# AI4Science-WestlakeU/safediffcon

Measured on AMD Instinct MI355X. Metric: sampled control trajectories/sec (1000-step DDPM), higher is better.
Workload: dtype f32; 1 GPU; C4: 2D smoke Unet3D_with_Conv3D dim=64 (1,2,4) state (B,32,7,64,64), B=64 per GPU, guided 1000-step DDPM, conformal quantile on; batch_per_gpu=64, global_batch=64, step=U-Net + guidance + posterior update of the whole batch, one hipGraph replay, parallelism=batch-sharded x1, no data-path collective, conv_precision=fp32

## Files before the change

include/sdc.h:

```cpp
#ifndef SDC_H
#define SDC_H

#include <stddef.h>
#include <stdint.h>

#ifdef __cplusplus
extern "C" {
#endif

#define SDC_OK 0
#define SDC_EINVAL (-1)
#define SDC_EALIGN (-2)
#define SDC_EHIP (-3)
#define SDC_ENULL (-4)

int sdc_version(void);
int sdc_last_error(char* buf, size_t cap);

typedef struct SdcConvDesc {
    int32_t B, Cin0, Cin1, Cout;
    int32_t iD, iH, iW;
    int32_t oD, oH, oW;
    int32_t kD, kH, kW;
    int32_t sD, sH, sW;
// ... 138 lines not shown
    int32_t pD, pH, pW;
    int32_t uD, uH, uW;
    int32_t precision;
    int64_t gs[5], xs[5];
} SdcWgradDesc;
size_t sdc_conv_wgrad_bytes(const SdcWgradDesc* d);
int sdc_conv_wgrad(const SdcWgradDesc* d, const float* g, const float* x, float* dw, float* dbias, void* work,
                   size_t work_bytes, void* stream);

#define SDC_F16_EXP_INTS 1025
int sdc_f16_grad_exponent(const float* g, int B, int C, int D, int H, int W, const int64_t* strides, int32_t* e, void* stream);

int sdc_conv_dgrad_f16(const SdcConvDesc* d, const float* g, const float* wp, const int32_t* e, float* dx, void* stream);

size_t sdc_conv_wgrad_f16_bytes(const SdcWgradDesc* d);
int sdc_conv_wgrad_f16(const SdcWgradDesc* d, const float* g, const float* x, const int32_t* e, float* dw, float* dbias, void* work,
                       size_t work_bytes, void* stream);
int sdc_conv_wgrad_describe(const SdcWgradDesc* d, char* name, size_t cap);

int sdc_conv_stem_f16_ok(const SdcConvDesc* d);
size_t sdc_pack_stem_f16_bytes(int Cout, int Cin, int kD, int kH, int kW);
int sdc_pack_stem_f16(const float* w, void* out, int Cout, int Cin, int kD, int kH, int kW, void* stream);
int sdc_conv_stem_f16(const SdcConvDesc* d, const float* x, const void* wh, const float* bias, float* y, void* stream);

int sdc_conv_stem_x3_ok(const SdcConvDesc* d);
size_t sdc_pack_stem_x3_bytes(int Cout, int Cin, int kD, int kH, int kW);
int sdc_pack_stem_x3(const float* w, void* out, int Cout, int Cin, int kD, int kH, int kW, void* stream);
int sdc_conv_stem_x3(const SdcConvDesc* d, const float* x, const void* wb, const float* bias, float* y, void* stream);

int sdc_conv_gemm_x3_ok(const SdcConvDesc* d);
size_t sdc_pack_gemm_x3_bytes(int Cout, int Cin, int kH, int kW);
int sdc_pack_gemm_x3(const float* wp, void* out, int Cout, int Cin, int kH, int kW, void* stream);
int sdc_conv_gemm_x3(const SdcConvDesc* d, const float* x, const void* wb, const float* bias, float* y, void* stream);

int sdc_conv_wino3_x3_ok(const SdcConvDesc* d);
size_t sdc_pack_wino3_x3_bytes(int Cout, int Cin);
int sdc_pack_wino3_x3(const float* wp, void* out, int Cout, int Cin, void* stream);
int sdc_conv_wino3_x3(const SdcConvDesc* d, const float* x, const float* x1, const void* wb, const float* bias, float* y,
                      double* gn_parts, int gn_groups, void* stream);

size_t sdc_gn_silu_bwd_floats(int B, int C, int G, int64_t S);
int sdc_gn_silu_bwd(const float* h, const float* gy, const float* stats, const float* gamma, const float* beta,
                    const float* ss, int64_t ss_b_stride, float* rows, float* gh, float* dgamma, float* dbeta, float* dss,
                    int B, int C, int G, int64_t S, void* stream);

size_t sdc_chan_norm_bwd_parts(int B, int64_t S);
size_t sdc_chan_norm_bwd_bytes(int B, int C, int64_t S);
int sdc_chan_norm_bwd(const float* x, const float* gy, const float* g, float* gx, float* gpart, int B, int C, int64_t S,
                      int mode, float eps, void* stream);

size_t sdc_pack_conv_weight_floats(int Cout, int Cin, int kD, int kH, int kW, int precision);
int sdc_pack_conv_weight(const float* w, float* out, int Cout, int Cin, int kD, int kH, int kW, int precision, int flip, void* stream);

typedef struct SdcPackItem {
    const float* w;
    float* out;
    int Cout, Cin, kD, kH, kW, precision, flip;
    int co_sh, ci_sh, grid_x, grid_y, block0;
    unsigned tap_magic;
    int64_t n[5];
} SdcPackItem;
int sdc_pack_batch_plan(SdcPackItem* items, int n, int* total_blocks, int* lds_bytes);
int sdc_pack_batch_run(const SdcPackItem* items_dev, int n, int total_blocks, int lds_bytes, void* stream);

size_t sdc_attn_bwd_bytes(int outer, int inner, int heads, int ntok);
int sdc_attn_bwd(const float* qkv, const float* dout, const float* rot, const float* bias, float* dqkv, float* dbias, void* work,
// ... 108 lines not shown
```

safediffcon_amd/_lib.py:

```python
import ctypes as C
import os

_HERE = os.path.dirname(os.path.abspath(__file__))
LIB_PATH = os.path.join(_HERE, "libsdc_hip.so")

SDC_MODEL_BURGERS, SDC_MODEL_TOKAMAK, SDC_MODEL_SMOKE = 0, 1, 2

_f32p = C.c_void_p
_i32p = C.c_void_p
_stream = C.c_void_p
_i64 = C.c_int64


class SdcConvDesc(C.Structure):
    _fields_ = [(n, C.c_int32) for n in (
        "B", "Cin0", "Cin1", "Cout", "iD", "iH", "iW", "oD", "oH", "oW", "kD", "kH", "kW", "sD", "sH", "sW",
        "pD", "pH", "pW", "uD", "uH", "uW", "up_mode", "precision")] + [
        ("x0s", C.c_int64 * 5), ("x1s", C.c_int64 * 5), ("ys", C.c_int64 * 5), ("rs", C.c_int64 * 5)]


class SdcStepDesc(C.Structure):
    _fields_ = [(n, C.c_int32) for n in (
        "model", "B", "d0", "d1", "d2", "d3", "guide", "clip", "impose", "cond_idx", "pad_zero", "use_max",
        "has_wgt", "skip_draws", "ddim")] + [("_pad", C.c_int32), ("seed", C.c_uint64)]
# ... 85 lines not shown
    "sdc_pack_tattn_x3": (C.c_int, [_f32p, _f32p, C.c_void_p, _stream]),
    "sdc_tattn_block_x3": (C.c_int, [_f32p, _f32p, C.c_void_p, _f32p, _f32p, _f32p, C.c_int, C.c_int, C.c_int, C.c_int,
                                     _i64, _i64, _i64, C.c_float, _stream]),
    "sdc_tattn_block_x3_ok": (C.c_int, [C.c_int, C.c_int, C.c_int]),
    "sdc_attn": (C.c_int, [_f32p, _f32p, _f32p, _f32p, C.c_int, C.c_int, C.c_int, C.c_int, _i64, _i64, _i64, _i64,
                           _i64, _i64, _i64, _i64, _stream]),
    "sdc_act": (C.c_int, [_f32p, _f32p, _i64, C.c_int, _stream]),
    "sdc_guide_reduce": (C.c_int, [C.POINTER(SdcStepDesc), _f32p, _f32p, _f32p, _i32p, _f32p, _f32p, _stream]),
    "sdc_step_update": (C.c_int, [C.POINTER(SdcStepDesc), _f32p, _f32p, _f32p, _f32p, _i32p, _i32p, _f32p, _i64,
                                  _f32p, _f32p, _f32p, _f32p, _f32p, _f32p, _f32p, _f32p, _stream]),
    "sdc_impose": (C.c_int, [C.POINTER(SdcStepDesc), _f32p, _f32p, _f32p, _f32p, _stream]),
    "sdc_randn": (C.c_int, [_f32p, _i64, C.c_uint64, _i32p, _stream]),
    "sdc_advance": (C.c_int, [_i32p, C.c_int, _i32p, C.c_int, _stream]),
    "sdc_advance_table": (C.c_int, [_i32p, _i32p, _i32p, _i32p, C.c_int, _stream]),
    "sdc_conformal_score": (C.c_int, [C.POINTER(SdcStepDesc), _f32p, _f32p, _f32p, _f32p, _f32p, _f32p, _stream]),
    "sdc_burgers_rollout": (C.c_int, [_f32p, _f32p, _f32p, C.c_int, C.c_int, C.c_int, C.c_int, C.c_int, C.c_float, C.c_float,
                                      C.c_float, C.c_float, C.c_float, _stream]),
    "sdc_conv_wgrad_bytes": (C.c_size_t, [C.POINTER(SdcWgradDesc)]),
    "sdc_conv_wgrad": (C.c_int, [C.POINTER(SdcWgradDesc), _f32p, _f32p, _f32p, _f32p, C.c_void_p, C.c_size_t, _stream]),
    "sdc_f16_grad_exponent": (C.c_int, [_f32p, C.c_int, C.c_int, C.c_int, C.c_int, C.c_int, C.c_void_p, C.c_void_p, _stream]),
    "sdc_conv_dgrad_f16": (C.c_int, [C.POINTER(SdcConvDesc), _f32p, _f32p, C.c_void_p, _f32p, _stream]),
    "sdc_conv_stem_f16_ok": (C.c_int, [C.POINTER(SdcConvDesc)]),
    "sdc_pack_stem_f16_bytes": (C.c_size_t, [C.c_int, C.c_int, C.c_int, C.c_int, C.c_int]),
    "sdc_pack_stem_f16": (C.c_int, [_f32p, C.c_void_p, C.c_int, C.c_int, C.c_int, C.c_int, C.c_int, _stream]),
    "sdc_conv_stem_f16": (C.c_int, [C.POINTER(SdcConvDesc), _f32p, C.c_void_p, _f32p, _f32p, _stream]),
    "sdc_conv_stem_x3_ok": (C.c_int, [C.POINTER(SdcConvDesc)]),
    "sdc_pack_stem_x3_bytes": (C.c_size_t, [C.c_int, C.c_int, C.c_int, C.c_int, C.c_int]),
    "sdc_pack_stem_x3": (C.c_int, [_f32p, C.c_void_p, C.c_int, C.c_int, C.c_int, C.c_int, C.c_int, _stream]),
    "sdc_conv_stem_x3": (C.c_int, [C.POINTER(SdcConvDesc), _f32p, C.c_void_p, _f32p, _f32p, _stream]),
    "sdc_conv_gemm_x3_ok": (C.c_int, [C.POINTER(SdcConvDesc)]),
    "sdc_pack_gemm_x3_bytes": (C.c_size_t, [C.c_int, C.c_int, C.c_int, C.c_int]),
    "sdc_pack_gemm_x3": (C.c_int, [_f32p, C.c_void_p, C.c_int, C.c_int, C.c_int, C.c_int, _stream]),
    "sdc_conv_gemm_x3": (C.c_int, [C.POINTER(SdcConvDesc), _f32p, C.c_void_p, _f32p, _f32p, _stream]),
    "sdc_conv_wino3_x3_ok": (C.c_int, [C.POINTER(SdcConvDesc)]),
    "sdc_pack_wino3_x3_bytes": (C.c_size_t, [C.c_int, C.c_int]),
    "sdc_pack_wino3_x3": (C.c_int, [_f32p, C.c_void_p, C.c_int, C.c_int, _stream]),
    "sdc_conv_wino3_x3": (C.c_int, [C.POINTER(SdcConvDesc), _f32p, _f32p, C.c_void_p, _f32p, _f32p, C.c_void_p, C.c_int, _stream]),
    "sdc_conv_wgrad_f16_bytes": (C.c_size_t, [C.POINTER(SdcWgradDesc)]),
    "sdc_conv_wgrad_f16": (C.c_int, [C.POINTER(SdcWgradDesc), _f32p, _f32p, C.c_void_p, _f32p, _f32p, C.c_void_p, C.c_size_t, _stream]),
    "sdc_conv_wgrad_describe": (C.c_int, [C.POINTER(SdcWgradDesc), C.c_char_p, C.c_size_t]),
    "sdc_gn_silu_bwd_floats": (C.c_size_t, [C.c_int, C.c_int, C.c_int, _i64]),
    "sdc_gn_silu_bwd": (C.c_int, [_f32p, _f32p, _f32p, _f32p, _f32p, _f32p, _i64, _f32p, _f32p, _f32p, _f32p, _f32p,
                                  C.c_int, C.c_int, C.c_int, _i64, _stream]),
    "sdc_chan_norm_bwd_parts": (C.c_size_t, [C.c_int, _i64]),
    "sdc_chan_norm_bwd_bytes": (C.c_size_t, [C.c_int, C.c_int, _i64]),
    "sdc_chan_norm_bwd": (C.c_int, [_f32p, _f32p, _f32p, _f32p, _f32p, C.c_int, C.c_int, _i64, C.c_int, C.c_float, _stream]),
    "sdc_pack_conv_weight_floats": (C.c_size_t, [C.c_int, C.c_int, C.c_int, C.c_int, C.c_int, C.c_int]),
    "sdc_pack_conv_weight": (C.c_int, [_f32p, _f32p, C.c_int, C.c_int, C.c_int, C.c_int, C.c_int, C.c_int, C.c_int, _stream]),
    "sdc_pack_batch_plan": (C.c_int, [C.POINTER(SdcPackItem), C.c_int, C.POINTER(C.c_int), C.POINTER(C.c_int)]),
    "sdc_pack_batch_run": (C.c_int, [C.c_void_p, C.c_int, C.c_int, C.c_int, _stream]),
    "sdc_attn_bwd_bytes": (C.c_size_t, [C.c_int, C.c_int, C.c_int, C.c_int]),
    "sdc_attn_bwd": (C.c_int, [_f32p, _f32p, _f32p, _f32p, _f32p, _f32p, C.c_void_p, C.c_int, C.c_int, C.c_int, C.c_int,
                               _i64, _i64, _i64, _i64, _i64, _i64, _i64, _i64, _stream]),
    "sdc_linattn_bwd_bytes": (C.c_size_t, [C.c_int, C.c_int, C.c_int, _i64]),
    "sdc_linattn_bwd": (C.c_int, [_f32p, _f32p, _f32p, C.c_void_p, C.c_int, C.c_int, C.c_int, _i64, _i64, _i64, _i64, _i64, _i64, _i64,
                                  _stream]),
    "sdc_act_bwd": (C.c_int, [_f32p, _f32p, _f32p, _i64, C.c_int, _stream]),
    "sdc_sumpool2": (C.c_int, [_f32p, _f32p, _i64, C.c_int, C.c_int, C.c_int, C.c_int, _stream]),
    "sdc_kstar_lstm_floats": (C.c_size_t, []),
    "sdc_kstar_rollout": (C.c_int, [C.POINTER(SdcKstarModel), _f32p, _i64, _i64, _i64, C.c_void_p, C.c_void_p, C.c_int, C.c_int, _stream]),
    "sdc_smoke_rollout_workspace_bytes": (C.c_size_t, [C.c_int]),
    "sdc_smoke_rollout": (C.c_int, [_f32p, _f32p, _i64, _i64, _f32p, _i64, _f32p, _i64, C.c_void_p, C.c_void_p, C.c_void_p,
                                    C.c_int, C.c_int, C.c_void_p, C.c_void_p, C.c_void_p, C.c_size_t, C.c_int, C.c_int, C.c_int,
                                    C.c_int, C.c_int, C.c_int, C.c_double, C.c_int, _stream]),
    "sdc_conv_splitk_bytes": (C.c_size_t, [C.POINTER(SdcConvDesc)]),
    "sdc_conv_splitk": (C.c_int, [C.POINTER(SdcConvDesc), _f32p, _f32p, _f32p, _f32p, _f32p, _f32p, C.c_size_t, _stream]),
# ... 57 lines not shown
```

safediffcon_amd/build.py:

```python
import os
import subprocess
import sys

HERE = os.path.dirname(os.path.abspath(__file__))
CSRC = os.path.join(HERE, "csrc")
LIB = os.path.join(HERE, "libsdc_hip.so")
SOURCES = ["sdc_api.hip", "sdc_conv.hip", "sdc_conv_wino.hip", "sdc_conv_f16.hip", "sdc_conv_stem_f16.hip", "sdc_conv_stem_x3.hip", "sdc_conv_gemm_x3.hip", "sdc_conv_wino_x3.hip", "sdc_norm.hip", "sdc_attn.hip", "sdc_lablock.hip", "sdc_lablock_f16.hip", "sdc_lablock_x3.hip", "sdc_tablock.hip", "sdc_tablock_f16.hip", "sdc_tablock_x3.hip", "sdc_step.hip", "sdc_solver.hip", "sdc_grad.hip", "sdc_wgrad_f16.hip", "sdc_attn_bwd.hip", "sdc_kstar.hip", "sdc_smoke.hip", "sdc_linear.hip", "sdc_optim.hip"]
HEADERS = ["sdc_common.h", "sdc_lablock_tile.h", "sdc_tablock_tile.h", "sdc_conv_stem_tile.h", "sdc_split3.h", "sdc_f16frag.h", "sdc_conv.h", "sdc_conv_wino3s.inc", "sdc_conv_wino2s.inc", "sdc_conv_pw2.inc"]
HIPCC = os.environ.get("HIPCC", "/opt/rocm/bin/hipcc")
FLAGS = ["--offload-arch=gfx950", "-O3", "-fPIC", "-std=c++17", "-Wall", "-Wno-unused-function"]


def source_hash():
    import hashlib
    h = hashlib.sha256()
    for f in SOURCES + HEADERS:
        with open(os.path.join(CSRC, f), "rb") as fh:
            h.update(fh.read())
    with open(os.path.join(HERE, "..", "include", "sdc.h"), "rb") as fh:
        h.update(fh.read())
    return h.hexdigest()[:16]


def _stale(out, deps):
    if not os.path.exists(out):
        return True
    t = os.path.getmtime(out)
    return any(os.path.getmtime(d) > t for d in deps)


def build_experiments(verbose=True):
    out = os.path.join(HERE, "libsdc_hip_exp.so")
    cmd = [HIPCC, *FLAGS, "-DSDC_KERNEL_EXPERIMENTS", "-shared", *[os.path.join(CSRC, s) for s in SOURCES], "-o", out]
    if verbose:
        print(" ".join(cmd), flush=True)
    subprocess.check_call(cmd)
    return out


def build(force=False, verbose=True, jobs=4):
# ... 28 lines not shown
```

safediffcon_amd/csrc/sdc_conv.h:

```cpp
#pragma once
#include "sdc_common.h"
#include <cstdlib>
#include <type_traits>

namespace sdcconv {


#ifdef SDC_KERNEL_EXPERIMENTS
inline int exp_env(const char* name) { const char* v = getenv(name); return v ? atoi(v) : 0; }
#else
constexpr int exp_env(const char*) { return 0; }
#endif


constexpr int BK = 16;
constexpr int NT = 256;

typedef float f32x16 __attribute__((ext_vector_type(16)));

typedef const __attribute__((address_space(1))) float* gfloat_p;
__device__ __forceinline__ gfloat_p uniform_ptr(const float* p) {
    const uint64_t u = reinterpret_cast<uint64_t>(p);
    const uint32_t lo = __builtin_amdgcn_readfirstlane((uint32_t)u);
    const uint32_t hi = __builtin_amdgcn_readfirstlane((uint32_t)(u >> 32));
// ... 38 lines not shown
constexpr int W3S_TILES = 32;

inline int64_t span5(const int64_t* st, int b, int c, int dd, int h, int w) {
    return (int64_t)(b - 1) * st[0] + (int64_t)(c - 1) * st[1] + (int64_t)(dd - 1) * st[2] + (int64_t)(h - 1) * st[3] + (int64_t)(w - 1) * st[4];
}

bool wg2_ok(const SdcConvDesc& d, bool small);
bool wg3_ok(const SdcConvDesc& d, bool small);
int launch_wg2(const ConvArgs& a, hipStream_t s);
int wg2_ksplit(const SdcConvDesc& d);
int launch_wg3(const ConvArgs& a, hipStream_t s);
bool wg3s_ok(const SdcConvDesc& d, bool small);
bool wg2s_ok(const SdcConvDesc& d, bool small);
int launch_wg2s(const ConvArgs& a, hipStream_t s);
int launch_wg3s(const ConvArgs& a, hipStream_t s);

int f16_kc(int kD, int kH, int kW);
bool f16_faster(const SdcConvDesc& d);
bool f16_ok(const SdcConvDesc& d);
int f16_gnparts(const SdcConvDesc& d, int G);
const char* f16_name(const SdcConvDesc& d);
int launch_f16(const ConvArgs& a, const _Float16* wh, hipStream_t s, const int32_t* gexp = nullptr);
int pack_f16_tail(const float* w, float* tail, int64_t gap, int Cout, int Cin, int kD, int kH, int kW, hipStream_t s);

struct StemShape { int Hs, NG, NR, itemsB; size_t lds; };
StemShape stem_shape(const SdcConvDesc& d);
int launch_stem_f16(const SdcConvDesc& d, const float* x, const _Float16* wh, const float* bias, float* y, hipStream_t s);

int launch_stem_x3(const SdcConvDesc& d, const float* x, const __bf16* wb, const float* bias, float* y, hipStream_t s);

bool gemm_x3_covers(const SdcConvDesc& d);
int launch_gemm_x3(const SdcConvDesc& d, const float* x, const __bf16* wb, const float* bias, float* y, hipStream_t s);

}
```

safediffcon_amd/csrc/sdc_conv.hip:

```cpp
#include "sdc_conv.h"
#include <string>

using namespace sdcconv;

namespace {

template <int TM, int TN>
__device__ __forceinline__ void conv_epilogue(const ConvArgs& a, f32x16 (&acc)[TM][TN], int mw, int nw, int lane, float* ybase = nullptr) {
    const SdcConvDesc& d = a.d;
    float* const ay = ybase ? ybase : a.y;
    const int l31 = lane & 31, lh = lane >> 5;
    if (a.ydense && mw + TM * 32 <= d.Cout) {
        typedef __attribute__((address_space(1))) char* gwchar_p;
        typedef __attribute__((address_space(1))) float* gwfloat_p;
        typedef const __attribute__((address_space(1))) char* gchar_p;
        const int S = d.oD * d.oH * d.oW;
        const float r_S = 1.0f / (float)S;
        const int64_t ycs4 = d.ys[1] * 4, rcs4 = d.rs[1] * 4;
        uint32_t yoff[TN], roff[TN];
        bool pok[TN];
#pragma unroll
        for (int j = 0; j < TN; ++j) {
            const int pp = nw + j * 32 + l31;
            pok[j] = pp < a.Ntot;
// ... 1474 lines not shown
        return (int64_t)(b - 1) * st[0] + (int64_t)(dd - 1) * st[2] + (int64_t)(h - 1) * st[3] + (int64_t)(w - 1) * st[4];
    };
    return span(d.x0s, d.B, d.iD, d.iH, d.iW) < (1ll << 30) && (d.Cin1 == 0 || span(d.x1s, d.B, d.iD, d.iH, d.iW) < (1ll << 30));
}

bool y_dense(const SdcConvDesc& d, bool residual) {
    auto dense = [&](const int64_t* st) { return st[4] == 1 && st[3] == d.oW && st[2] == (int64_t)d.oH * d.oW; };
    const int64_t S = (int64_t)d.oD * d.oH * d.oW;
    return dense(d.ys) && S >= 128 && S < (1 << 24) && span5(d.ys, d.B, d.Cout, d.oD, d.oH, d.oW) < (1ll << 30) &&
           (!residual || (dense(d.rs) && span5(d.rs, d.B, d.Cout, d.oD, d.oH, d.oW) < (1ll << 30)));
}

struct Operands { const void *x0, *x1, *wp, *y, *res; };
const void* const ALIGNED = reinterpret_cast<const void*>(uintptr_t(256));
const Operands CANONICAL{ALIGNED, ALIGNED, ALIGNED, ALIGNED, nullptr};

bool aligned(const void* p, int bytes) { return reinterpret_cast<uintptr_t>(p) % bytes == 0; }

bool wino_aligned(const SdcConvDesc& d, const Operands& op, bool stores) {
    return aligned(op.wp, 16) && aligned(op.x0, 16) && (d.Cin1 == 0 || aligned(op.x1, 16)) && (!stores || (aligned(op.y, 8) && !op.res));
}

std::string wino_misfit(const SdcConvDesc& d, const Operands& op) {
    std::string s;
    auto add = [&](bool miss, const char* what) { if (miss) s += (s.empty() ? "" : ", ") + std::string(what); };
    add(!aligned(op.wp, 16), "wp is not 16-byte aligned");
    add(!aligned(op.x0, 16), "x0 is not 16-byte aligned");
    add(d.Cin1 > 0 && !aligned(op.x1, 16), "x1 is not 16-byte aligned");
    add(!aligned(op.y, 8), "y is not 8-byte aligned");
    add(op.res != nullptr, "a residual is fused");
    return s.empty() ? "the operands differ from the descriptor-only assumption" : s;
}

enum class Kern { F16, WG3S, WG3, WG2S, WG2, WG1, PW2, PW, STEM, DIRECT };
struct Route {
    Kern kern;
    const char* name;
    double share;
    int gn_parts;
    int ksplit;
    bool sum_bias;
    int tile;
    bool ups;
    Direct form;
};

Route make_route(Kern k, const char* name, double share, int gn_parts = 0, int tile = 0) {
    return Route{k, name, share, gn_parts, 1, false, tile, false, Direct::GEN};
}

Route route(const SdcConvDesc& d, const Operands& op, int G, bool split) {
    if (d.precision == 6 || d.precision == 7) {
        if (!split && f16_ok(d)) return make_route(Kern::F16, f16_name(d), 1.0, f16_gnparts(d, G));
        SdcConvDesc d4 = d;
        d4.precision = 4;
        return route(d4, op, G, split);
    }
    const bool small = conv_small(d);
    const int64_t ntot = (int64_t)d.B * d.oD * d.oH * d.oW;
    const bool splits = split && !op.res;
    if (wg3s_ok(d, small) && wino_aligned(d, op, true))
        return make_route(Kern::WG3S, d.oW == 16 ? "conv_wg3s_kernel<16>" : (d.oW == 32 ? "conv_wg3s_kernel<32>" : "conv_wg3s_kernel<64>"),
                          8.0 / 27.0, gn_parts_for(d, W2_BM, W3S_TILES * 8, G));
    if (wg3_ok(d, small) && wino_aligned(d, op, true))
        return make_route(Kern::WG3, d.oW == 16 ? "conv_wg3_kernel<16>" : (d.oW == 32 ? "conv_wg3_kernel<32>" : "conv_wg3_kernel<64>"),
                          8.0 / 27.0, gn_parts_for(d, W2_BM, W2_TILES * 8, G));
    if (wg2s_ok(d, small) && wino_aligned(d, op, true) && !(split && wg2_ksplit(d) > 1))
        return make_route(Kern::WG2S, d.oW == 128 ? "conv_wg2s_kernel<128>" : (d.oW == 64 ? "conv_wg2s_kernel<64>" : "conv_wg2s_kernel<32>"),
                          4.0 / 9.0, gn_parts_for(d, W2_BM, W3S_TILES * 4, G));
    if (wg2_ok(d, small) && wino_aligned(d, op, false)) {
        Route r = make_route(Kern::WG2, d.oW == 16 ? "conv_wg2_kernel<16>" : (d.oW == 32 ? "conv_wg2_kernel<32>" :
                                        (d.oW == 64 ? "conv_wg2_kernel<64>" : "conv_wg2_kernel<128>")), 4.0 / 9.0,
                             gn_parts_for(d, W2_BM, W2_TILES * 4, G));
        r.ksplit = splits ? wg2_ksplit(d) : 1;
        return r;
    }
    const WgPick w = wg_pick(d, ntot, small);
    if (w.pick && aligned(op.wp, 16)) {
        const char* name;
        if (w.ups) name = w.pick == 6 ? "conv_wg_kernel<128,128,4,2,16,512,ups>" : (w.pick == 7 ? "conv_wg_kernel<64,256,2,4,16,512,ups>" :
                                                                                     "conv_wg_kernel<64,128,2,2,16,256,ups>");
        else name = w.pick == 13 ? "conv_f43_kernel<128,128,4,16,F43>" : w.pick == 6 ? "conv_wg_kernel<128,128,4,2,16,512>" :
                    w.pick == 7 ? "conv_wg_kernel<64,256,2,4,16,512>" : w.pick == 9 ? "conv_wg_kernel<128,256,4,2,16,512>" :
                    w.pick == 10 ? "conv_wg_kernel<64,512,1,8,16,512>" : "conv_wg_kernel<64,128,2,2,16,512,ks2>";
        Route r = make_route(Kern::WG1, name, w.pick == 13 ? 0.5 : 2.0 / 3.0, gn_parts_for(d, w.bm, w.bn, G), w.pick);
        r.ups = w.ups;
        r.ksplit = (splits && d.oW % 4 == 0 && d.ys[4] == 1) ? wg1_ksplit(d, w, ntot) : 1;
        r.sum_bias = true;
        return r;
    }
    const bool fast = (d.Cin0 % BK == 0) && (d.Cin1 % BK == 0) && small && d.Cout < (1 << 30);
    auto direct = [&](int t) {
        const DirectTile& T = DIRECT_TILES[t];
        const bool rh = T.bm >= 64 && fast && d.sW == 1 && d.uD == 1 && d.uH == 1 && d.uW == 1 && d.up_mode == 0 &&
                        d.kW == 3 && d.kD * d.kH <= 32 && d.Cout % 4 == 0 &&
                        ((d.oW % T.bn == 0) || (T.bn % d.oW == 0 && d.oW >= 16)) && aligned(op.wp, 16);
        Route r = make_route(Kern::DIRECT, nullptr, 1.0, 0, t);
        r.form = rh ? Direct::RH : (fast ? Direct::FAST : Direct::GEN);
        r.name = T.names[(int)r.form];
        return r;
    };
    auto dense_in = [&](const int64_t* st) { return st[4] == 1 && st[3] == d.iW && st[2] == (int64_t)d.iH * d.iW && st[0] % 4 == 0 && st[1] % 4 == 0; };
    const bool pw = fast && d.kD * d.kH * d.kW == 1 && d.sD == 1 && d.sH == 1 && d.sW == 1 && d.uD == 1 && d.uH == 1 &&
        d.uW == 1 && d.up_mode == 0 && d.pD == 0 && d.pH == 0 && d.pW == 0 && d.oD == d.iD && d.oH == d.iH && d.oW == d.iW &&
        (int64_t)d.oD * d.oH * d.oW % 4 == 0 && d.Cout % 4 == 0 && d.Cout > 32 && dense_in(d.x0s) && (d.Cin1 == 0 || dense_in(d.x1s)) &&
        aligned(op.x0, 16) && (d.Cin1 == 0 || aligned(op.x1, 16)) && aligned(op.wp, 16);
    const int sd = (splits && d.oW % 4 == 0 && d.precision != 5) ? direct_ksplit(d, ntot, fast) : 1;
    if (sd > 1) {
        Route r = pw ? make_route(Kern::PW, "conv_pw_kernel<64,64,2,2>", 1.0, 0, 3) : direct(3);
        r.ksplit = sd;
        r.sum_bias = true;
        return r;
    }
    if (pw) {
        const bool al16 = aligned(op.y, 16) && d.ys[0] % 4 == 0 && d.ys[1] % 4 == 0 &&
                          (!op.res || (aligned(op.res, 16) && d.rs[0] % 4 == 0 && d.rs[1] % 4 == 0));
        const bool pw2 = al16 && y_dense(d, op.res != nullptr);
        if (pw2 && d.Cout % 128 == 0 && ((ntot + 255) / 256) * (d.Cout / 128) >= 1024) return make_route(Kern::PW2, "conv_pw2_kernel<2,2>", 1.0, 0, 0);
        if (pw2 && d.Cout == 64 && (ntot + 511) / 512 >= 1024) return make_route(Kern::PW2, "conv_pw2_kernel<1,4>", 1.0, 0, 1);
        if (d.Cout > 64 && ntot >= 128 * 256) return make_route(Kern::PW, "conv_pw_kernel<128,128,2,2>", 1.0, 0, 0);
        if (d.Cout <= 64 && ntot >= 256 * 1024) return make_route(Kern::PW, "conv_pw_kernel<64,256,1,4>", 1.0, 0, 1);
        if (((ntot + 127) / 128) * ((d.Cout + 63) / 64) >= 1024) return make_route(Kern::PW, "conv_pw_kernel<64,128,2,2>", 1.0, 0, 2);
        return make_route(Kern::PW, "conv_pw_kernel<64,64,2,2>", 1.0, 0, 3);
    }
    if (d.kW == 7 && d.sW == 1 && d.uD == 1 && d.uH == 1 && d.uW == 1 && d.up_mode == 0 && d.kD * d.kH <= 64 &&
        d.Cout % 4 == 0 && d.Cout > 32 && small && ((d.oW % 128 == 0) || (128 % d.oW == 0 && d.oW >= 16)) && aligned(op.wp, 16))
        return make_route(Kern::STEM, "conv_rh_kernel<64,128,2,2,7,true>", 1.0);
    if (d.Cout > 64 && ntot >= 128 * 256) return direct(0);
    if (d.Cout > 32 && d.Cout <= 64 && ntot >= 256 * 1024) return direct(1);
    if (d.Cout > 32 && ((ntot + 127) / 128) * ((d.Cout + 63) / 64) >= 1024) return direct(2);
    if (d.Cout > 32) return direct(3);
    return direct(4);
}

bool stem_f16_ok(const SdcConvDesc& d) {
    if (!(d.kW == 7 && ((d.kD == 1 && (d.kH == 1 || d.kH == 7)) || (d.kD == 7 && d.kH == 7)))) return false;
    if (!(d.sD == 1 && d.sH == 1 && d.sW == 1 && d.uD == 1 && d.uH == 1 && d.uW == 1 && d.up_mode == 0)) return false;
    if (!(d.pW == 3 && d.pH == d.kH / 2 && d.pD == d.kD / 2 && d.oD == d.iD && d.oH == d.iH && d.oW == d.iW)) return false;
    if (!(d.B > 0 && d.oD > 0 && d.oH > 0 && d.Cin0 >= 1 && d.Cin0 <= 8 && d.Cin1 == 0 && d.Cout > 0 && d.Cout % 64 == 0)) return false;
    if (!(d.oW == 16 || d.oW == 32 || d.oW == 64 || d.oW == 128)) return false;
    return d.x0s[4] == 1 && d.ys[4] == 1;
}

__global__ __launch_bounds__(256) void splitk_sum_kernel(const float* __restrict__ part, float* __restrict__ y, int S, int64_t elems, int C,
                                                         int oD, int oH, int oW, int64_t s0, int64_t s1, int64_t s2, int64_t s3, int64_t s4,
                                                         const float* __restrict__ bias = nullptr) {
    typedef float nf4 __attribute__((ext_vector_type(4)));
    const int64_t q = (int64_t)blockIdx.x * 256 + threadIdx.x;
    if (q * 4 >= elems) return;
    nf4 acc = *reinterpret_cast<const nf4*>(part + q * 4);
// ... 45 lines not shown
                "sdc_conv_dgrad_f16: precision 6 or 7, one input");
    return conv_impl(dp, g, nullptr, wp, nullptr, nullptr, dx, nullptr, 0, stream, nullptr, 0, e);
}

extern "C" size_t sdc_conv_splitk_bytes(const SdcConvDesc* dp) {
    if (!dp) return 0;
    const SdcConvDesc& d = *dp;
    const int S = route(d, CANONICAL, 0, true).ksplit;
    return S > 1 ? (size_t)S * d.B * d.Cout * d.oD * d.oH * d.oW * sizeof(float) : 0;
}

extern "C" int sdc_conv_splitk(const SdcConvDesc* dp, const float* x0, const float* x1, const float* wp, const float* bias, float* y,
                               float* work, size_t work_bytes, void* stream) {
    return conv_impl(dp, x0, x1, wp, bias, nullptr, y, nullptr, 0, stream, work, work_bytes);
}

extern "C" int sdc_conv_gnparts(const SdcConvDesc* dp, int G) {
    return dp ? route(*dp, CANONICAL, G, false).gn_parts : 0;
}

extern "C" int sdc_conv_gn(const SdcConvDesc* dp, const float* x0, const float* x1, const float* wp, const float* bias,
                           const float* residual, float* y, double* parts, int G, void* stream) {
    SDC_REQUIRE(parts && G > 0, SDC_EINVAL, "sdc_conv_gn: parts buffer and a positive group count are required");
    return conv_impl(dp, x0, x1, wp, bias, residual, y, parts, G, stream);
}

extern "C" int sdc_conv_describe(const SdcConvDesc* dp, char* name, size_t cap, double* mfma_share) {
    SDC_REQUIRE(dp, SDC_ENULL, "sdc_conv_describe: null descriptor");
    { const int rc = check_conv(*dp, CANONICAL, false); if (rc != SDC_OK) return rc; }
    const Route r = route(*dp, CANONICAL, 0, false);
    if (name && cap) { std::strncpy(name, r.name, cap - 1); name[cap - 1] = 0; }
    if (mfma_share) *mfma_share = r.share;
    return SDC_OK;
}

extern "C" int sdc_conv_stem_f16_ok(const SdcConvDesc* dp) {
    return dp && stem_f16_ok(*dp) ? 1 : 0;
}

extern "C" int sdc_conv_stem_f16(const SdcConvDesc* dp, const float* x, const void* wh, const float* bias, float* y, void* stream) {
    SDC_REQUIRE(dp && x && wh && y, SDC_ENULL, "sdc_conv_stem_f16: null pointer");
    SDC_REQUIRE(stem_f16_ok(*dp), SDC_EINVAL, "sdc_conv_stem_f16: descriptor not covered (sdc_conv_stem_f16_ok returned 0): %dx%dx%d taps, Cin %d+%d, "
                "Cout %d, rows of %d", dp->kD, dp->kH, dp->kW, dp->Cin0, dp->Cin1, dp->Cout, dp->oW);
    return launch_stem_f16(*dp, x, reinterpret_cast<const _Float16*>(wh), bias, y, sdc::as_stream(stream));
}

extern "C" int sdc_conv_stem_x3_ok(const SdcConvDesc* dp) {
    return dp && stem_f16_ok(*dp) && dp->kD == 7 ? 1 : 0;
}

extern "C" int sdc_conv_stem_x3(const SdcConvDesc* dp, const float* x, const void* wb, const float* bias, float* y, void* stream) {
    SDC_REQUIRE(dp && x && wb && y, SDC_ENULL, "sdc_conv_stem_x3: null pointer");
    SDC_REQUIRE(stem_f16_ok(*dp), SDC_EINVAL, "sdc_conv_stem_x3: descriptor not covered (sdc_conv_stem_f16_ok returned 0): %dx%dx%d taps, Cin %d+%d, "
                "Cout %d, rows of %d", dp->kD, dp->kH, dp->kW, dp->Cin0, dp->Cin1, dp->Cout, dp->oW);
    return launch_stem_x3(*dp, x, reinterpret_cast<const __bf16*>(wb), bias, y, sdc::as_stream(stream));
}

namespace {

int conv_impl(const SdcConvDesc* dp, const float* x0, const float* x1, const float* wp, const float* bias,
              const float* residual, float* y, double* gn_part, int gn_G, void* stream, float* split_work, size_t split_bytes,
              const int32_t* gexp) {
    SDC_REQUIRE(dp && x0 && wp && y, SDC_ENULL, "sdc_conv: null pointer");
    const SdcConvDesc& d = *dp;
    const Operands op{x0, x1, wp, y, residual};
    { const int rc = check_conv(d, op, gn_part != nullptr); if (rc != SDC_OK) return rc; }
// ... 23 lines not shown
    if (r.ksplit > 1) {
        SDC_REQUIRE(split_bytes >= (size_t)r.ksplit * elems * sizeof(float), SDC_EINVAL, "sdc_conv_splitk: workspace too small");
        SDC_REQUIRE(aligned(split_work, 16), SDC_EINVAL, "sdc_conv_splitk: workspace must be 16-byte aligned");
        SDC_REQUIRE(elems <= (1ll << 30), SDC_EINVAL, "sdc_conv_splitk: partial copy too large");
        a.ksplit = r.ksplit; a.ypart_elems = elems; a.y = split_work;
        a.d.ys[4] = 1; a.d.ys[3] = d.oW; a.d.ys[2] = (int64_t)d.oH * d.oW; a.d.ys[1] = a.d.ys[2] * d.oD; a.d.ys[0] = a.d.ys[1] * d.Cout;
        a.vec2 = 1;
        a.ydense = (int64_t)d.oD * d.oH * d.oW >= 128 && (int64_t)d.oD * d.oH * d.oW < (1 << 24);
        if (r.sum_bias) a.bias = nullptr;
    }
    hipStream_t s = sdc::as_stream(stream);
    const float* const taps2 = wp + (int64_t)a.Ktot * d.Cout + (int64_t)(a.Ktot / 3 * 4) * d.Cout;
    int rc = SDC_OK;
    switch (r.kern) {
        case Kern::F16: {
            const size_t off = (sdc_pack_conv_weight_floats(d.Cout, a.Cin, d.kD, d.kH, d.kW, 4) + 3) & ~(size_t)3;
            return launch_f16(a, reinterpret_cast<const _Float16*>(wp + off), s, gexp);
        }
        case Kern::WG3S: a.wg2 = taps2 + (int64_t)(a.Ktot / 9 * 16) * d.Cout; rc = launch_wg3s(a, s); break;
        case Kern::WG3: a.wg2 = taps2 + (int64_t)(a.Ktot / 9 * 16) * d.Cout; rc = launch_wg3(a, s); break;
        case Kern::WG2S: a.wg2 = taps2; rc = launch_wg2s(a, s); break;
        case Kern::WG2: a.wg2 = taps2; a.lgW = ilog2_pow2(d.oW); rc = launch_wg2(a, s); break;
        case Kern::WG1:
            switch (r.tile) {
                case 13: rc = launch_f43<128, 128, 4, 16>(a, s); break;
                case 6: rc = r.ups ? launch_wg<128, 128, 4, 2, 16, 512, true>(a, s) : launch_wg<128, 128, 4, 2, 16, 512>(a, s); break;
                case 7: rc = r.ups ? launch_wg<64, 256, 2, 4, 16, 512, true>(a, s) : launch_wg<64, 256, 2, 4, 16, 512>(a, s); break;
                case 9: rc = launch_wg<128, 256, 4, 2, 16, 512>(a, s); break;
                case 10: rc = launch_wg<64, 512, 1, 8, 16, 512>(a, s); break;
                default:
                    rc = r.ups ? launch_wg<64, 128, 2, 2, 16, 256, true>(a, s) : launch_wg<64, 128, 2, 2, 16, 512, false, 4, 2>(a, s);
            }
            break;
        case Kern::PW2: rc = r.tile == 0 ? launch_pw2<2, 2>(a, s) : launch_pw2<1, 4>(a, s); break;
        case Kern::PW:
            switch (r.tile) {
                case 0: launch_pw<128, 128, 2, 2>(a, s); break;
                case 1: launch_pw<64, 256, 1, 4>(a, s); break;
                case 2: launch_pw<64, 128, 2, 2>(a, s); break;
                default: launch_pw<64, 64, 2, 2>(a, s);
            }
            break;
        case Kern::STEM:
            hipLaunchKernelGGL((conv_rh_kernel<64, 128, 2, 2, 7, true, 8>), dim3((a.Ntot + 127) / 128, (d.Cout + 63) / 64), dim3(NT), 0, s, a);
            break;
        case Kern::DIRECT:
            switch (r.tile) {
                case 0: launch_direct<128, 128, 2, 2>(a, r.form, s); break;
                case 1: launch_direct<64, 256, 1, 4>(a, r.form, s); break;
                case 2: launch_direct<64, 128, 2, 2>(a, r.form, s); break;
                case 3: launch_direct<64, 64, 2, 2>(a, r.form, s); break;
                default: launch_direct<32, 128, 1, 4>(a, r.form, s);
            }
            break;
    }
    if (rc != SDC_OK) return rc;
    if (r.ksplit > 1)
        hipLaunchKernelGGL(splitk_sum_kernel, dim3((unsigned)((elems / 4 + 255) / 256)), dim3(256), 0, s, (const float*)split_work, y, r.ksplit,
                           elems, d.Cout, d.oD, d.oH, d.oW, d.ys[0], d.ys[1], d.ys[2], d.ys[3], d.ys[4], r.sum_bias ? bias : nullptr);
    const hipError_t e = hipGetLastError();
    SDC_REQUIRE(e == hipSuccess, SDC_EHIP, "%s[%s]: %s", r.ksplit > 1 ? "sdc_conv_splitk" : "sdc_conv", r.name, hipGetErrorString(e));
    return SDC_OK;
}

}
```

Measured before the change: 0.3104 trajectories/s.

## Add bf16x3-split MFMA pointwise conv kernel for selected 1x1x1 shapes

Adds a persistent 1x1x1 convolution kernel that splits fp32 weights and activations into three bf16 pieces and accumulates six bf16 MFMA products to emulate fp32 accuracy. The weight block stays resident in LDS while each wave walks position tiles, with global loads, splitting and LDS reads software-pipelined against the MFMAs. The router sends a hardcoded table of channel and spatial shapes to this kernel whenever precision is not 2 or 3, replacing the existing fp32 pointwise kernels for those shapes. In exchange it adds split overhead and a bf16x3 approximation of fp32 arithmetic on the routed shapes.

```diff
diff --git a/include/sdc.h b/include/sdc.h
--- a/include/sdc.h
+++ b/include/sdc.h
@@ -194,6 +194,10 @@
 size_t sdc_pack_gemm_x3_bytes(int Cout, int Cin, int kH, int kW);
 int sdc_pack_gemm_x3(const float* wp, void* out, int Cout, int Cin, int kH, int kW, void* stream);
 int sdc_conv_gemm_x3(const SdcConvDesc* d, const float* x, const void* wb, const float* bias, float* y, void* stream);
+
+int sdc_conv_pw_x3_ok(const SdcConvDesc* d);
+int sdc_conv_pw_x3(const SdcConvDesc* d, const float* x0, const float* x1, const float* wp, const float* bias, const float* residual,
+                   float* y, void* stream);
 
 int sdc_conv_wino3_x3_ok(const SdcConvDesc* d);
 size_t sdc_pack_wino3_x3_bytes(int Cout, int Cin);
diff --git a/safediffcon_amd/_lib.py b/safediffcon_amd/_lib.py
--- a/safediffcon_amd/_lib.py
+++ b/safediffcon_amd/_lib.py
@@ -141,6 +141,8 @@
     "sdc_pack_gemm_x3_bytes": (C.c_size_t, [C.c_int, C.c_int, C.c_int, C.c_int]),
     "sdc_pack_gemm_x3": (C.c_int, [_f32p, C.c_void_p, C.c_int, C.c_int, C.c_int, C.c_int, _stream]),
     "sdc_conv_gemm_x3": (C.c_int, [C.POINTER(SdcConvDesc), _f32p, C.c_void_p, _f32p, _f32p, _stream]),
+    "sdc_conv_pw_x3_ok": (C.c_int, [C.POINTER(SdcConvDesc)]),
+    "sdc_conv_pw_x3": (C.c_int, [C.POINTER(SdcConvDesc), _f32p, _f32p, _f32p, _f32p, _f32p, _f32p, _stream]),
     "sdc_conv_wino3_x3_ok": (C.c_int, [C.POINTER(SdcConvDesc)]),
     "sdc_pack_wino3_x3_bytes": (C.c_size_t, [C.c_int, C.c_int]),
     "sdc_pack_wino3_x3": (C.c_int, [_f32p, C.c_void_p, C.c_int, C.c_int, _stream]),
diff --git a/safediffcon_amd/build.py b/safediffcon_amd/build.py
--- a/safediffcon_amd/build.py
+++ b/safediffcon_amd/build.py
@@ -5,7 +5,7 @@
 HERE = os.path.dirname(os.path.abspath(__file__))
 CSRC = os.path.join(HERE, "csrc")
 LIB = os.path.join(HERE, "libsdc_hip.so")
-SOURCES = ["sdc_api.hip", "sdc_conv.hip", "sdc_conv_wino.hip", "sdc_conv_f16.hip", "sdc_conv_stem_f16.hip", "sdc_conv_stem_x3.hip", "sdc_conv_gemm_x3.hip", "sdc_conv_wino_x3.hip", "sdc_norm.hip", "sdc_attn.hip", "sdc_lablock.hip", "sdc_lablock_f16.hip", "sdc_lablock_x3.hip", "sdc_tablock.hip", "sdc_tablock_f16.hip", "sdc_tablock_x3.hip", "sdc_step.hip", "sdc_solver.hip", "sdc_grad.hip", "sdc_wgrad_f16.hip", "sdc_attn_bwd.hip", "sdc_kstar.hip", "sdc_smoke.hip", "sdc_linear.hip", "sdc_optim.hip"]
+SOURCES = ["sdc_api.hip", "sdc_conv.hip", "sdc_conv_wino.hip", "sdc_conv_f16.hip", "sdc_conv_stem_f16.hip", "sdc_conv_stem_x3.hip", "sdc_conv_gemm_x3.hip", "sdc_conv_pw_x3.hip", "sdc_conv_wino_x3.hip", "sdc_norm.hip", "sdc_attn.hip", "sdc_lablock.hip", "sdc_lablock_f16.hip", "sdc_lablock_x3.hip", "sdc_tablock.hip", "sdc_tablock_f16.hip", "sdc_tablock_x3.hip", "sdc_step.hip", "sdc_solver.hip", "sdc_grad.hip", "sdc_wgrad_f16.hip", "sdc_attn_bwd.hip", "sdc_kstar.hip", "sdc_smoke.hip", "sdc_linear.hip", "sdc_optim.hip"]
 HEADERS = ["sdc_common.h", "sdc_lablock_tile.h", "sdc_tablock_tile.h", "sdc_conv_stem_tile.h", "sdc_split3.h", "sdc_f16frag.h", "sdc_conv.h", "sdc_conv_wino3s.inc", "sdc_conv_wino2s.inc", "sdc_conv_pw2.inc"]
 HIPCC = os.environ.get("HIPCC", "/opt/rocm/bin/hipcc")
 FLAGS = ["--offload-arch=gfx950", "-O3", "-fPIC", "-std=c++17", "-Wall", "-Wno-unused-function"]
diff --git a/safediffcon_amd/csrc/sdc_conv.h b/safediffcon_amd/csrc/sdc_conv.h
--- a/safediffcon_amd/csrc/sdc_conv.h
+++ b/safediffcon_amd/csrc/sdc_conv.h
@@ -94,4 +94,7 @@
 bool gemm_x3_covers(const SdcConvDesc& d);
 int launch_gemm_x3(const SdcConvDesc& d, const float* x, const __bf16* wb, const float* bias, float* y, hipStream_t s);
 
+int pw_x3_block(int K, int Cout);
+int launch_pw_x3(const ConvArgs& a, hipStream_t s);
+
 }
diff --git a/safediffcon_amd/csrc/sdc_conv.hip b/safediffcon_amd/csrc/sdc_conv.hip
--- a/safediffcon_amd/csrc/sdc_conv.hip
+++ b/safediffcon_amd/csrc/sdc_conv.hip
@@ -1530,7 +1530,7 @@
     return s.empty() ? "the operands differ from the descriptor-only assumption" : s;
 }
 
-enum class Kern { F16, WG3S, WG3, WG2S, WG2, WG1, PW2, PW, STEM, DIRECT };
+enum class Kern { F16, WG3S, WG3, WG2S, WG2, WG1, PWX3, PW2, PW, STEM, DIRECT };
 struct Route {
     Kern kern;
     const char* name;
@@ -1545,6 +1545,43 @@
 
 Route make_route(Kern k, const char* name, double share, int gn_parts = 0, int tile = 0) {
     return Route{k, name, share, gn_parts, 1, false, tile, false, Direct::GEN};
+}
+
+bool pw_dense(const SdcConvDesc& d, const Operands& op) {
+    const bool fast = (d.Cin0 % BK == 0) && (d.Cin1 % BK == 0) && conv_small(d) && d.Cout < (1 << 30);
+    auto dense_in = [&](const int64_t* st) { return st[4] == 1 && st[3] == d.iW && st[2] == (int64_t)d.iH * d.iW && st[0] % 4 == 0 && st[1] % 4 == 0; };
+    return fast && d.kD * d.kH * d.kW == 1 && d.sD == 1 && d.sH == 1 && d.sW == 1 && d.uD == 1 && d.uH == 1 &&
+        d.uW == 1 && d.up_mode == 0 && d.pD == 0 && d.pH == 0 && d.pW == 0 && d.oD == d.iD && d.oH == d.iH && d.oW == d.iW &&
+        (int64_t)d.oD * d.oH * d.oW % 4 == 0 && d.Cout % 4 == 0 && d.Cout > 32 && dense_in(d.x0s) && (d.Cin1 == 0 || dense_in(d.x1s)) &&
+        aligned(op.x0, 16) && (d.Cin1 == 0 || aligned(op.x1, 16)) && aligned(op.wp, 16);
+}
+
+bool pw_dense_out(const SdcConvDesc& d, const Operands& op) {
+    const bool al16 = aligned(op.y, 16) && d.ys[0] % 4 == 0 && d.ys[1] % 4 == 0 &&
+                      (!op.res || (aligned(op.res, 16) && d.rs[0] % 4 == 0 && d.rs[1] % 4 == 0));
+    return al16 && y_dense(d, op.res != nullptr);
+}
+
+bool pw_x3_covers(const SdcConvDesc& d, const Operands& op) {
+    const int K = d.Cin0 + d.Cin1;
+    auto lane_span = [&](const int64_t* st) { return (int64_t)(d.B - 1) * st[0] + (int64_t)d.oD * d.oH * d.oW + 16 * st[1] < (1ll << 30); };
+    return pw_dense(d, op) && pw_dense_out(d, op) && K >= 64 && K % 32 == 0 && pw_x3_block(K, d.Cout) > 0 &&
+           lane_span(d.x0s) && (d.Cin1 == 0 || lane_span(d.x1s));
+}
+
+const char* pw_x3_name(int mb) { return mb == 128 ? "conv_pw_x3_kernel<4,2>" : mb == 96 ? "conv_pw_x3_kernel<3,2>" : "conv_pw_x3_kernel<2,2>"; }
+
+bool pw_x3_faster(const SdcConvDesc& d) {
+    struct Row { int cin0, cin1, cout, S; };
+    static const Row rows[] = {
+        {128, 0, 384, 32 * 32 * 32}, {256, 0, 384, 32 * 16 * 16}, {128, 0, 256, 32 * 16 * 16}, {64, 64, 64, 32 * 64 * 64},
+        {128, 0, 128, 32 * 32 * 32}, {128, 128, 64, 32 * 32 * 32}, {128, 0, 384, 32 * 16 * 16}, {64, 0, 128, 32 * 32 * 32},
+        {128, 0, 128, 32 * 16 * 16},
+    };
+    const int64_t S = (int64_t)d.oD * d.oH * d.oW;
+    for (const Row& r : rows)
+        if (d.Cin0 == r.cin0 && d.Cin1 == r.cin1 && d.Cout == r.cout && S == r.S) return true;
+    return false;
 }
 
 Route route(const SdcConvDesc& d, const Operands& op, int G, bool split) {
@@ -1598,11 +1635,7 @@
         r.name = T.names[(int)r.form];
         return r;
     };
-    auto dense_in = [&](const int64_t* st) { return st[4] == 1 && st[3] == d.iW && st[2] == (int64_t)d.iH * d.iW && st[0] % 4 == 0 && st[1] % 4 == 0; };
-    const bool pw = fast && d.kD * d.kH * d.kW == 1 && d.sD == 1 && d.sH == 1 && d.sW == 1 && d.uD == 1 && d.uH == 1 &&
-        d.uW == 1 && d.up_mode == 0 && d.pD == 0 && d.pH == 0 && d.pW == 0 && d.oD == d.iD && d.oH == d.iH && d.oW == d.iW &&
-        (int64_t)d.oD * d.oH * d.oW % 4 == 0 && d.Cout % 4 == 0 && d.Cout > 32 && dense_in(d.x0s) && (d.Cin1 == 0 || dense_in(d.x1s)) &&
-        aligned(op.x0, 16) && (d.Cin1 == 0 || aligned(op.x1, 16)) && aligned(op.wp, 16);
+    const bool pw = pw_dense(d, op);
     const int sd = (splits && d.oW % 4 == 0 && d.precision != 5) ? direct_ksplit(d, ntot, fast) : 1;
     if (sd > 1) {
         Route r = pw ? make_route(Kern::PW, "conv_pw_kernel<64,64,2,2>", 1.0, 0, 3) : direct(3);
@@ -1611,9 +1644,9 @@
         return r;
     }
     if (pw) {
-        const bool al16 = aligned(op.y, 16) && d.ys[0] % 4 == 0 && d.ys[1] % 4 == 0 &&
-                          (!op.res || (aligned(op.res, 16) && d.rs[0] % 4 == 0 && d.rs[1] % 4 == 0));
-        const bool pw2 = al16 && y_dense(d, op.res != nullptr);
+        if (d.precision != 2 && d.precision != 3 && pw_x3_faster(d) && pw_x3_covers(d, op))
+            return make_route(Kern::PWX3, pw_x3_name(pw_x3_block(d.Cin0 + d.Cin1, d.Cout)), 0.0);
+        const bool pw2 = pw_dense_out(d, op);
         if (pw2 && d.Cout % 128 == 0 && ((ntot + 255) / 256) * (d.Cout / 128) >= 1024) return make_route(Kern::PW2, "conv_pw2_kernel<2,2>", 1.0, 0, 0);
         if (pw2 && d.Cout == 64 && (ntot + 511) / 512 >= 1024) return make_route(Kern::PW2, "conv_pw2_kernel<1,4>", 1.0, 0, 1);
         if (d.Cout > 64 && ntot >= 128 * 256) return make_route(Kern::PW, "conv_pw_kernel<128,128,2,2>", 1.0, 0, 0);
@@ -1725,6 +1758,33 @@
     if (name && cap) { std::strncpy(name, r.name, cap - 1); name[cap - 1] = 0; }
     if (mfma_share) *mfma_share = r.share;
     return SDC_OK;
+}
+
+extern "C" int sdc_conv_pw_x3_ok(const SdcConvDesc* dp) {
+    if (!dp || check_conv(*dp, CANONICAL, false) != SDC_OK) return 0;
+    Operands op = CANONICAL;
+    if (dp->rs[1] != 0) op.res = ALIGNED;
+    return pw_x3_faster(*dp) && pw_x3_covers(*dp, op) ? 1 : 0;
+}
+
+extern "C" int sdc_conv_pw_x3(const SdcConvDesc* dp, const float* x0, const float* x1, const float* wp, const float* bias,
+                              const float* residual, float* y, void* stream) {
+    SDC_REQUIRE(dp && x0 && wp && y, SDC_ENULL, "sdc_conv_pw_x3: null pointer");
+    const SdcConvDesc& d = *dp;
+    const Operands op{x0, x1, wp, y, residual};
+    { const int rc = check_conv(d, op, false); if (rc != SDC_OK) return rc; }
+    SDC_REQUIRE(pw_x3_covers(d, op), SDC_EINVAL, "sdc_conv_pw_x3: descriptor not covered: %dx%dx%d taps, stride %dx%dx%d, Cin %d+%d, Cout %d, "
+                "output %dx%dx%d (1x1x1 stride-1 convs over dense 16-byte aligned operands, Cin a multiple of 32 from 64 to 256, Cout a "
+                "multiple of 64 or 96, the weight block within the LDS: include/sdc.h)", d.kD, d.kH, d.kW, d.sD, d.sH, d.sW, d.Cin0, d.Cin1, d.Cout,
+                d.oD, d.oH, d.oW);
+    ConvArgs a{};
+    a.d = d;
+    a.x0 = x0; a.x1 = x1; a.wp = wp; a.bias = bias; a.res = residual; a.y = y;
+    a.Ntot = d.B * d.oD * d.oH * d.oW;
+    a.Cin = d.Cin0 + d.Cin1;
+    a.Ktot = a.Cin;
+    a.ksplit = 1;
+    return launch_pw_x3(a, sdc::as_stream(stream));
 }
 
 extern "C" int sdc_conv_stem_f16_ok(const SdcConvDesc* dp) {
@@ -1814,6 +1874,7 @@
                     rc = r.ups ? launch_wg<64, 128, 2, 2, 16, 256, true>(a, s) : launch_wg<64, 128, 2, 2, 16, 512, false, 4, 2>(a, s);
             }
             break;
+        case Kern::PWX3: rc = launch_pw_x3(a, s); break;
         case Kern::PW2: rc = r.tile == 0 ? launch_pw2<2, 2>(a, s) : launch_pw2<1, 4>(a, s); break;
         case Kern::PW:
             switch (r.tile) {
diff --git a/safediffcon_amd/csrc/sdc_conv_pw_x3.hip b/safediffcon_amd/csrc/sdc_conv_pw_x3.hip
--- /dev/null
+++ b/safediffcon_amd/csrc/sdc_conv_pw_x3.hip
@@ -0,0 +1,271 @@
+#include "sdc_conv.h"
+#include "sdc_split3.h"
+
+namespace sdc { int ta_grid(const char* entry, int64_t nblk, unsigned* grid); }
+
+using namespace sdcconv;
+
+namespace {
+
+constexpr int PX_NT = 256;
+constexpr int PX_LDS_MAX = 160 * 1024;
+
+struct PwX3Args {
+    const float *x0, *x1, *wp, *bias, *res;
+    float* y;
+    int64_t x0s1, x1s1, ys1, rs1;
+    int x0s0, x1s0, ys0, rs0;
+    int Cin0, K, Cout, S, Ntot;
+    int ntiles, MT, nwalk, gx;
+};
+
+template <int TM, int TN, bool RES>
+__global__ __launch_bounds__(PX_NT) __attribute__((amdgpu_waves_per_eu(1))) SDC_NO_DS_MERGE void conv_pw_x3_kernel(const PwX3Args a) {
+    constexpr int MB = 32 * TM, WP = 32 * TN;
+    static_assert(TN == 2 || TN == 4, "position tiles per wave");
+    typedef float vecn __attribute__((ext_vector_type(TN)));
+    typedef float nfloat4 __attribute__((ext_vector_type(4)));
+    typedef const __attribute__((address_space(1))) vecn* gvec_p;
+    typedef __attribute__((address_space(1))) vecn* gwvec_p;
+    typedef const __attribute__((address_space(1))) char* gchar_p;
+    typedef __attribute__((address_space(1))) char* gwchar_p;
+    extern __shared__ __attribute__((aligned(16))) char px_lds[];
+
+    const int tid = threadIdx.x, lane = tid & 63, wave = SDC_UNIFORM(tid >> 6);
+    const int l31 = lane & 31, lh = lane >> 5;
+    const int K = a.K, nch = K >> 4;
+    const int PSZ = K * MB * 2;
+    int mt, walker;
+    if (a.gx) {
+        const int q = blockIdx.x >> 3;
+        mt = q % a.MT;
+        walker = (blockIdx.x & 7) * (a.gx / a.MT) + q / a.MT;
+    } else {
+        mt = blockIdx.x % a.MT;
+        walker = blockIdx.x / a.MT;
+    }
+    const int m0 = mt * MB;
+
+    for (int e = tid; e < (K >> 3) * MB; e += PX_NT) {
+        const int oct = e / MB, co = e - oct * MB;
+        const float* w = a.wp + (int64_t)(oct * 8) * a.Cout + m0 + co;
+        float v[8];
+#pragma unroll
+        for (int j = 0; j < 8; ++j) v[j] = w[(int64_t)j * a.Cout];
+        bf16x8 h, m, l;
+        split3x8(v, h, m, l);
+        *reinterpret_cast<bf16x8*>(px_lds + e * 16) = h;
+        *reinterpret_cast<bf16x8*>(px_lds + PSZ + e * 16) = m;
+        *reinterpret_cast<bf16x8*>(px_lds + 2 * PSZ + e * 16) = l;
+    }
+    float* const lbias = reinterpret_cast<float*>(px_lds + 3 * PSZ);
+    if (tid < MB) lbias[tid] = a.bias ? a.bias[m0 + tid] : 0.0f;
+    __syncthreads();
+
+    const int nww = a.nwalk * 4;
+    const int t_first = walker * 4 + wave;
+    auto tile_off = [&](const int t, uint32_t& o0, uint32_t& o1) {
+        const int p = t < a.ntiles ? t * WP + TN * l31 : a.Ntot;
+        const int pp = p < a.Ntot ? p : 0;
+        const int b = pp / a.S, sp = pp - b * a.S;
+        o0 = (uint32_t)(b * a.x0s0 + sp + 8 * lh * (int)a.x0s1) * 4u;
+        o1 = K > a.Cin0 ? (uint32_t)(b * a.x1s0 + sp + 8 * lh * (int)a.x1s1) * 4u : 0u;
+    };
+    int l_c = 0;
+    uint32_t l_o0, l_o1, n_o0 = 0, n_o1 = 0;
+    tile_off(t_first, l_o0, l_o1);
+    vecn raw[2][8];
+    auto issue = [&](const int set) __attribute__((always_inline)) {
+        const int ci = l_c * 16;
+        const bool first = ci < a.Cin0;
+        const int64_t cs = first ? a.x0s1 : a.x1s1;
+        const gchar_p base = (gchar_p)uniform_ptr(first ? a.x0 + ci * cs : a.x1 + (ci - a.Cin0) * cs);
+        const uint32_t cs4 = (uint32_t)cs * 4u;
+        uint32_t o = first ? l_o0 : l_o1;
+#pragma unroll
+        for (int j = 0; j < 8; ++j) {
+            raw[set][j] = *(gvec_p)(base + o);
+            o += cs4;
+        }
+        const bool wrap = ++l_c == nch;
+        l_c = wrap ? 0 : l_c;
+        l_o0 = wrap ? n_o0 : l_o0;
+        l_o1 = wrap ? n_o1 : l_o1;
+    };
+
+    bf16x8 a0[2][TM], a1[TM], a2[TM], bfr[2][TN][3];
+    const int a_lane = (lh * MB + l31) * 16;
+    auto read_a = [&](bf16x8 (&dst)[TM], const int piece, const int c) __attribute__((always_inline)) {
+#pragma unroll
+        for (int i = 0; i < TM; ++i)
+            dst[i] = *reinterpret_cast<const bf16x8*>(px_lds + piece * PSZ + (c * 2 * MB + 32 * i) * 16 + a_lane);
+    };
+    auto split_part = [&](const int set, const int part) __attribute__((always_inline)) {
+        const int j = part >> 1, kh = part & 1;
+#pragma unroll
+        for (int k = 4 * kh; k < 4 * kh + 4; ++k) {
+            __bf16 ph, pm, pl;
+            split3(raw[set][k][j], ph, pm, pl);
+            bfr[set][j][0][k] = ph; bfr[set][j][1][k] = pm; bfr[set][j][2][k] = pl;
+        }
+    };
+
+    f32x16 acc[TM][TN], sm[TM][TN];
+    auto step = [&](auto pc, auto fc, auto lc, const int c) __attribute__((always_inline)) {
+        constexpr int P = decltype(pc)::value;
+        constexpr bool FIRST = decltype(fc)::value, LAST = decltype(lc)::value;
+        const int cn = c + 1 == nch ? 0 : c + 1;
+#pragma unroll
+        for (int t = 0; t < 6; ++t) {
+#pragma unroll
+            for (int i = 0; i < TM; ++i)
+#pragma unroll
+                for (int j = 0; j < TN; ++j) {
+                    f32x16& c16 = t < 5 ? sm[i][j] : acc[i][j];
+                    f32x16 cin = c16;
+                    if (FIRST && (t == 0 || t == 5)) {
+#pragma unroll
+                        for (int r = 0; r < 16; ++r) cin[r] = 0.0f;
+                    }
+                    const bf16x8 av = X3_PA[t] == 0 ? a0[P][i] : (X3_PA[t] == 1 ? a1[i] : a2[i]);
+                    c16 = __builtin_amdgcn_mfma_f32_32x32x16_bf16(av, bfr[P][j][X3_PB[t]], cin, 0, 0, 0);
+                }
+            if (!LAST) {
+                if (t == 0) read_a(a2, 2, cn);
+                if (t == 1) read_a(a0[P ^ 1], 0, cn);
+                if (t == 3) read_a(a1, 1, cn);
+            }
+            if (t < 4) {
+#pragma unroll
+                for (int q = 0; q < TN / 2; ++q) split_part(P ^ 1, t * (TN / 2) + q);
+            }
+            if (t == 5) issue(P ^ 1);
+            __builtin_amdgcn_sched_barrier(0);
+        }
+    };
+
+    issue(0);
+    issue(1);
+#pragma unroll
+    for (int q = 0; q < 2 * TN; ++q) split_part(0, q);
+    issue(0);
+    read_a(a2, 2, 0);
+    read_a(a1, 1, 0);
+    read_a(a0[0], 0, 0);
+
+    constexpr std::integral_constant<int, 0> P0{};
+    constexpr std::integral_constant<int, 1> P1{};
+    for (int t = t_first; t < a.ntiles; t += nww) {
+        tile_off(t + nww, n_o0, n_o1);
+        constexpr std::true_type Y{};
+        constexpr std::false_type N{};
+        step(P0, Y, N, 0);
+        step(P1, N, N, 1);
+        for (int c = 2; c + 2 < nch; c += 2) {
+            step(P0, N, N, c);
+            step(P1, N, N, c + 1);
+        }
+        step(P0, N, N, nch - 2);
+        step(P1, N, Y, nch - 1);
+        const int p = t * WP + TN * l31;
+        const bool pok = p < a.Ntot;
+        const int pp = pok ? p : 0;
+        const int b = pp / a.S, sp = pp - b * a.S;
+        uint32_t yo = (uint32_t)(b * a.ys0 + sp + 4 * lh * (int)a.ys1) * 4u;
+        uint32_t ro = RES ? (uint32_t)(b * a.rs0 + sp + 4 * lh * (int)a.rs1) * 4u : 0u;
+        const uint32_t ys4 = (uint32_t)a.ys1 * 4u, rs4 = (uint32_t)a.rs1 * 4u;
+        const gchar_p rb = (gchar_p)uniform_ptr(RES ? a.res + (int64_t)m0 * a.rs1 : a.y);
+        const gwchar_p yb = (gwchar_p)(__attribute__((address_space(1))) void*)uniform_ptr(a.y + (int64_t)m0 * a.ys1);
+#pragma unroll
+        for (int i = 0; i < TM; ++i) {
+#pragma unroll
+            for (int hb = 0; hb < 2; ++hb) {
+                vecn rv[8];
+                nfloat4 bz[2];
+                if (RES) {
+#pragma unroll
+                    for (int q = 0; q < 8; ++q) {
+                        rv[q] = *(gvec_p)(rb + ro);
+                        ro += (q & 3) < 3 ? rs4 : 5 * rs4;
+                    }
+                }
+#pragma unroll
+                for (int g = 0; g < 2; ++g) bz[g] = *reinterpret_cast<const nfloat4*>(lbias + 32 * i + 8 * (2 * hb + g) + 4 * lh);
+                vecn v[8];
+#pragma unroll
+                for (int q = 0; q < 8; ++q) {
+                    const int rr = hb * 8 + q;
+#pragma unroll
+                    for (int j = 0; j < TN; ++j) v[q][j] = (acc[i][j][rr] + sm[i][j][rr]) + bz[q >> 2][q & 3];
+                    if (RES) v[q] += rv[q];
+                }
+                if (pok) {
+                    uint32_t o = yo;
+#pragma unroll
+                    for (int q = 0; q < 8; ++q) {
+                        *(gwvec_p)(yb + o) = v[q];
+                        o += (q & 3) < 3 ? ys4 : 5 * ys4;
+                    }
+                }
+                yo += 16 * ys4;
+                __builtin_amdgcn_sched_barrier(0);
+            }
+        }
+        read_a(a2, 2, 0);
+        read_a(a1, 1, 0);
+        read_a(a0[0], 0, 0);
+    }
+}
+
+template <int TM, int TN>
+int launch_px(PwX3Args& a, int ncu, hipStream_t s) {
+    constexpr int MB = 32 * TM, WP = 32 * TN;
+    a.ntiles = (a.Ntot + WP - 1) / WP;
+    a.MT = a.Cout / MB;
+    const int need = (a.ntiles + 3) / 4;
+    const int per = ncu / 8;
+    if (ncu % 8 == 0 && per >= a.MT && 8 * (per / a.MT) <= need) {
+        a.gx = (per / a.MT) * a.MT;
+        a.nwalk = 8 * (per / a.MT);
+    } else {
+        a.gx = 0;
+        a.nwalk = ncu / a.MT < 1 ? 1 : ncu / a.MT;
+        if (a.nwalk > need) a.nwalk = need;
+    }
+    const size_t lds = (size_t)3 * a.K * MB * 2 + MB * sizeof(float);
+    if (a.res) {
+        static std::atomic<uint64_t> attr{0};
+        SDC_LDS_OPTIN(attr, (conv_pw_x3_kernel<TM, TN, true>), PX_LDS_MAX, "sdc_conv_pw_x3");
+        hipLaunchKernelGGL((conv_pw_x3_kernel<TM, TN, true>), dim3((unsigned)(a.nwalk * a.MT)), dim3(PX_NT), lds, s, a);
+    } else {
+        static std::atomic<uint64_t> attr{0};
+        SDC_LDS_OPTIN(attr, (conv_pw_x3_kernel<TM, TN, false>), PX_LDS_MAX, "sdc_conv_pw_x3");
+        hipLaunchKernelGGL((conv_pw_x3_kernel<TM, TN, false>), dim3((unsigned)(a.nwalk * a.MT)), dim3(PX_NT), lds, s, a);
+    }
+    return sdc::check_launch("sdc_conv_pw_x3");
+}
+
+}
+
+namespace sdcconv {
+
+int pw_x3_block(int K, int Cout) {
+    for (const int mb : {128, 96, 64})
+        if (Cout % mb == 0 && (size_t)3 * K * mb * 2 + mb * sizeof(float) <= (size_t)PX_LDS_MAX) return mb;
+    return 0;
+}
+
+int launch_pw_x3(const ConvArgs& c, hipStream_t s) {
+    const SdcConvDesc& d = c.d;
+    PwX3Args a;
+    a.x0 = c.x0; a.x1 = c.x1; a.wp = c.wp; a.bias = c.bias; a.res = c.res; a.y = c.y;
+    a.x0s1 = d.x0s[1]; a.x1s1 = d.x1s[1]; a.ys1 = d.ys[1]; a.rs1 = d.rs[1];
+    a.x0s0 = d.B > 1 ? (int)d.x0s[0] : 0; a.x1s0 = d.B > 1 ? (int)d.x1s[0] : 0; a.ys0 = d.B > 1 ? (int)d.ys[0] : 0; a.rs0 = d.B > 1 ? (int)d.rs[0] : 0;
+    a.Cin0 = d.Cin0; a.K = d.Cin0 + d.Cin1; a.Cout = d.Cout; a.S = d.oD * d.oH * d.oW; a.Ntot = c.Ntot;
+    unsigned ncu = 0;
+    if (const int rc = sdc::ta_grid("sdc_conv_pw_x3", 1 << 30, &ncu)) return rc;
+    const int mb = pw_x3_block(a.K, a.Cout);
+    return mb == 128 ? launch_px<4, 2>(a, (int)ncu, s) : mb == 96 ? launch_px<3, 2>(a, (int)ncu, s) : launch_px<2, 2>(a, (int)ncu, s);
+}
+
+}
```

New measurement: 0.3144 trajectories/s (median of 6 runs). 1.01x the previous value.
